# sz3/libcimbar

Hardware: NVIDIA H100
Metric: decoded cimbar frames/sec (1024x1024 mode-B) (higher is better)
Workload: dtype u8 (integer/bitwise; float32 only in the colour classifier, bit-exact vs reference)

## Files before the change

### libcimbar_b200/csrc/api.cu

```cuda
#include "ctx.cuh"
#include "k1_decode.cuh"
#include "k2_rs.cuh"
#include "render.cuh"
#include "encode.cuh"

#include <atomic>
#include <cmath>
#include <cstdio>
#include <cstring>
#include <string>
#include <vector>

using namespace cb200;

namespace {

thread_local std::string g_err;
std::atomic<unsigned long long> g_launches{0};

}
namespace cb200 {
int fail(int code, const std::string& msg) { g_err = msg; return code; }
int fail_cuda(cudaError_t e, const char* what)
{
// ... 528 lines not shown
int cb200_destroy(cb200_ctx* c)
{
    if (!c) return CB200_OK;
    cudaSetDevice(c->device);
    for (int k = 0; k < cb200_ctx::kEvSets; ++k) for (int i = 0; i < 8; ++i) if (c->ev[k][i]) cudaEventDestroy(c->ev[k][i]);
    for (const auto& s : c->stage) if (s.ev) cudaEventDestroy(s.ev);
    if (c->ccm_ev) cudaEventDestroy(c->ccm_ev);
    gather_destroy(c->gather);
    deskew_destroy(c->deskew); scan_destroy(c->scan);
    if (c->own_stream) cudaStreamDestroy(c->own_stream);
    delete c;
    return CB200_OK;
}

int cb200_get_info(const cb200_ctx* c, cb200_info* out)
{
    if (!c || !out) return fail(CB200_ERR_ARG, "null argument");
    fill_info(c->mode, c->max_frames, c->sm_count, out);
    return CB200_OK;
}

int cb200_set_stream(cb200_ctx* c, void* cuda_stream)
{
    if (!c) return fail(CB200_ERR_ARG, "null context");
    c->stream = cuda_stream ? (cudaStream_t)cuda_stream : c->own_stream;
    return CB200_OK;
}

int cb200_sync(cb200_ctx* c)
{
    if (!c) return fail(CB200_ERR_ARG, "null context");
    CK(cudaStreamSynchronize(c->stream), "cudaStreamSynchronize");
    return CB200_OK;
}

int cb200_decode_raw_dev(cb200_ctx* c, const uint8_t* d_rgb, int n, uint32_t flags, uint8_t* d_raw_out, uint8_t* d_frame_flags)
{
    int rc = check_frame_flags(flags); if (rc) return rc;
    rc = check_n(c, n); if (rc) return rc;
    if (n == 0) return CB200_OK;
    if (!d_rgb || !d_raw_out) return fail(CB200_ERR_ARG, "null buffer");
    CK(cudaSetDevice(c->device), "cudaSetDevice");
    const uint16_t* idx;
    rc = idx_for(c, flags, &idx); if (rc) return rc;
    rc = run_cells(c, d_rgb, n, flags, nullptr); if (rc) return rc;
    CK(k2_pack_launch(c->mode, c->d_cellvals, idx, n, d_raw_out, c->stream), "pack launch");
    mark(c);
    if (d_frame_flags) CK(cudaMemcpyAsync(d_frame_flags, c->d_flags, (size_t)n, cudaMemcpyDeviceToDevice, c->stream), "copy flags");
    return CB200_OK;
}

int cb200_rs_correct_dev(cb200_ctx* c, const uint8_t* d_raw, int n, uint8_t* d_data_out, uint8_t* d_block_ok)
{
    int rc = check_n(c, n); if (rc) return rc;
    if (n == 0) return CB200_OK;
    if (!d_raw || !d_data_out) return fail(CB200_ERR_ARG, "null buffer");
    CK(cudaSetDevice(c->device), "cudaSetDevice");
    uint8_t* ok = d_block_ok ? d_block_ok : c->d_ok;
    CK(k2_rs_launch(c->mode, d_raw, n, d_data_out, ok, c->d_rho, c->sm_count, c->stream), "rs launch");
    return CB200_OK;
}

}

namespace {
int decode_chunks(cb200_ctx* c, const uint8_t* d_rgb, int n, uint32_t flags, const uint8_t* sharpen, uint8_t* d_chunks,
                  uint32_t* d_chunk_mask, uint8_t* d_frame_flags, const uint8_t* d_sel_bytes = nullptr, bool enqueue_only = false)
{
    int rc = check_n(c, n); if (rc) return rc;
    if (n == 0) return CB200_OK;
    if (!d_rgb || !d_chunks || !d_chunk_mask) return fail(CB200_ERR_ARG, "null buffer");
    CK(cudaSetDevice(c->device), "cudaSetDevice");
    const Mode& m = c->mode;
    if ((flags & CB200_FLAG_CC_FIT) && (flags & CB200_FLAG_CC_SIMPLE)) return fail(CB200_ERR_ARG, "CC_SIMPLE and CC_FIT are exclusive");
    const bool fit = (flags & CB200_FLAG_CC_FIT) && !m.legacy && m.ecc_bytes > 0 && m.color_bits > 0;
    bool carried = false;
    if (enqueue_only && !(flags & CB200_FLAG_CC_SIMPLE) && c->ccm_pending) {
        const cudaError_t q = cudaEventQuery(c->ccm_ev);
        if (q == cudaErrorNotReady) carried = true;
        else if (q != cudaSuccess) return fail_cuda(q, "query ccm");
    }
    const uint16_t* idx;
    rc = idx_for(c, flags, &idx); if (rc) return rc;
    if (!fit && !carried) {
        rc = run_cells(c, d_rgb, n, flags & ~CB200_FLAG_CC_FIT, sharpen, nullptr, nullptr, d_sel_bytes); if (rc) return rc;
        mark(c);
        CK(k2_rs_fused_launch(m, c->d_cellvals, idx, n, d_chunks, c->d_ok, c->d_rho, c->sm_count, c->stream), "rs launch");
    } else {
        rc = ccm_buffers(c); if (rc) return rc;
        CK(c->d_means.ensure((size_t)c->max_frames * m.num_cells), "cudaMalloc means");
        CK(c->d_ccm_active.ensure((size_t)c->max_frames), "cudaMalloc ccm flags");
        CcmArg initial;
        if (carried) {
            memset(&initial, 0, sizeof(initial));
            initial.per_frame = c->d_carry;
            initial.per_frame_active = reinterpret_cast<const uint8_t*>(c->d_carry + 9);
        } else {
            rc = ccm_arg(c, initial); if (rc) return rc;
        }
        rc = run_cells(c, d_rgb, n, flags & ~(CB200_FLAG_CC_FIT | CB200_FLAG_CC_SIMPLE), sharpen, nullptr, c->d_means, d_sel_bytes); if (rc) return rc;
        mark(c);
        if (fit) {
            CK(k2_rs_fused_launch(m, c->d_cellvals, idx, n, d_chunks, c->d_ok, c->d_rho, c->sm_count, c->stream, 0, m.nblocks_sym), "rs launch (symbols)");
            CK(ccm_fit_launch(m, d_rgb, d_chunks, c->d_ok, idx, n, c->d_fit, c->d_fit_valid, c->stream), "ccm fit");
        } else {
            CK(cudaMemsetAsync(c->d_fit_valid, 0, (size_t)n, c->stream), "memset fit flags");
        }
        CK(ccm_carry_launch(n, c->d_fit, c->d_fit_valid, initial, c->d_ccm, c->d_ccm_active, c->stream), "ccm carry");
        CK(ccm_apply_launch(m, c->d_means, n, c->d_ccm, c->d_ccm_active, c->d_cellvals, c->stream), "ccm apply");
        if (fit) {
            CK(k2_rs_fused_launch(m, c->d_cellvals, idx, n, d_chunks, c->d_ok, c->d_rho, c->sm_count, c->stream, m.nblocks_sym, m.nblocks - m.nblocks_sym),
               "rs launch (colours)");
            rc = ccm_keep_last(c, n, c->d_ccm_active); if (rc) return rc;
        } else {
            CK(k2_rs_fused_launch(m, c->d_cellvals, idx, n, d_chunks, c->d_ok, c->d_rho, c->sm_count, c->stream), "rs launch");
        }
    }
    mark(c);
    CK(k2_mask_launch(m, c->d_ok, n, d_chunk_mask, c->stream), "mask launch");
    mark(c);
    if (d_frame_flags) CK(cudaMemcpyAsync(d_frame_flags, c->d_flags, (size_t)n, cudaMemcpyDeviceToDevice, c->stream), "copy flags");
    return CB200_OK;
}
}

extern "C" {

int cb200_decode_chunks_dev(cb200_ctx* c, const uint8_t* d_rgb, int n, uint32_t flags, uint8_t* d_chunks, uint32_t* d_chunk_mask, uint8_t* d_frame_flags)
{
    int rc = check_frame_flags(flags); if (rc) return rc;
    return decode_chunks(c, d_rgb, n, flags, nullptr, d_chunks, d_chunk_mask, d_frame_flags);
}

int cb200_decode_chunks_sharpen_dev(cb200_ctx* c, const uint8_t* d_rgb, int n, uint32_t flags, const uint8_t* sharpen, uint8_t* d_chunks,
                                    uint32_t* d_chunk_mask, uint8_t* d_frame_flags)
{
    int rc = check_selection_args(flags, sharpen); if (rc) return rc;
    return decode_chunks(c, d_rgb, n, flags, sharpen, d_chunks, d_chunk_mask, d_frame_flags);
}

int cb200_decode_raw(cb200_ctx* c, const uint8_t* rgb, int n, uint32_t flags, uint8_t* raw_out, uint8_t* frame_flags)
{
    int rc = check_frame_flags(flags); if (rc) return rc;
    rc = check_n(c, n); if (rc) return rc;
    if (n == 0) return CB200_OK;
    if (!rgb || !raw_out) return fail(CB200_ERR_ARG, "null buffer");
    CK(cudaSetDevice(c->device), "cudaSetDevice");
    rc = upload_frames(c, rgb, n); if (rc) return rc;
    rc = cb200_decode_raw_dev(c, c->d_rgb, n, flags, c->d_raw, nullptr); if (rc) return rc;
    CK(cudaMemcpyAsync(raw_out, c->d_raw, (size_t)n * c->mode.cap_all, cudaMemcpyDeviceToHost, c->stream), "D2H raw");
    if (frame_flags) CK(cudaMemcpyAsync(frame_flags, c->d_flags, (size_t)n, cudaMemcpyDeviceToHost, c->stream), "D2H flags");
    CK(cudaStreamSynchronize(c->stream), "sync");
    return CB200_OK;
}

int cb200_decode(cb200_ctx* c, const uint8_t* rgb, int n, uint32_t flags, uint8_t* data_out, uint8_t* block_ok, uint8_t* frame_flags)
{
    int rc = check_frame_flags(flags); if (rc) return rc;
    rc = check_n(c, n); if (rc) return rc;
    if (n == 0) return CB200_OK;
    if (!rgb || !data_out) return fail(CB200_ERR_ARG, "null buffer");
    CK(cudaSetDevice(c->device), "cudaSetDevice");
    rc = upload_frames(c, rgb, n); if (rc) return rc;
    rc = cb200_decode_chunks_dev(c, c->d_rgb, n, flags, c->d_data, c->d_mask, nullptr); if (rc) return rc;
    CK(cudaMemcpyAsync(data_out, c->d_data, (size_t)n * c->mode.data_bytes, cudaMemcpyDeviceToHost, c->stream), "D2H data");
    if (block_ok) CK(cudaMemcpyAsync(block_ok, c->d_ok, (size_t)n * c->mode.nblocks, cudaMemcpyDeviceToHost, c->stream), "D2H ok");
    if (frame_flags) CK(cudaMemcpyAsync(frame_flags, c->d_flags, (size_t)n, cudaMemcpyDeviceToHost, c->stream), "D2H flags");
    CK(cudaStreamSynchronize(c->stream), "sync");
    return CB200_OK;
}

}

namespace {
int decode_fountain_from_host(cb200_ctx* c, const uint8_t* rgb, int n, uint32_t flags, const uint8_t* sharpen, uint8_t* chunks_out,
                              uint32_t* chunk_count, uint32_t* chunk_mask, uint8_t* frame_flags)
{
    int rc = check_n(c, n); if (rc) return rc;
    if (n == 0) return CB200_OK;
    if (!rgb || !chunks_out || !chunk_count) return fail(CB200_ERR_ARG, "null buffer");
    CK(cudaSetDevice(c->device), "cudaSetDevice");
    rc = upload_frames(c, rgb, n); if (rc) return rc;
    return decode_fountain_to_host(c, c->d_rgb, n, flags, sharpen, chunks_out, chunk_count, chunk_mask, frame_flags);
}
}

int cb200::decode_fountain_to_host(cb200_ctx* c, const uint8_t* d_rgb, int n, uint32_t flags, const uint8_t* sharpen, uint8_t* chunks_out,
                                   uint32_t* chunk_count, uint32_t* chunk_mask, uint8_t* frame_flags)
{
    int rc = check_n(c, n); if (rc) return rc;
    if (n == 0) return CB200_OK;
    if (!d_rgb || !chunks_out || !chunk_count) return fail(CB200_ERR_ARG, "null buffer");
    CK(cudaSetDevice(c->device), "cudaSetDevice");
    rc = decode_chunks(c, d_rgb, n, flags, sharpen, c->d_data, c->d_mask, nullptr); if (rc) return rc;
    return fetch_fountain(c, n, nullptr, chunks_out, chunk_count, chunk_mask, frame_flags, nullptr);
}

int cb200::decode_chunks_enqueue(cb200_ctx* c, const uint8_t* d_rgb, int n, uint32_t flags, const uint8_t* d_sharp, uint8_t* d_chunks,
// ... 220 lines not shown
```

### libcimbar_b200/csrc/k2_rs.cu

```cuda
#include "cb200_common.cuh"
#include "k2_rs.cuh"
#include <cstring>
#include <cstdint>

namespace cb200 {

constexpr int kMaxParity = 64;

__constant__ uint8_t c_gf_exp[512];
__constant__ uint8_t c_gf_log[256];

__device__ __forceinline__ uint32_t slot_value(const uint8_t* __restrict__ cells, const uint16_t* __restrict__ idx,
                                               uint32_t s, int stream, int symbol_bits)
{
    uint32_t v = cells[idx[s]] & 0x7Fu;
    uint32_t sym_mask = (1u << symbol_bits) - 1u;
    if (stream == 0) return v & sym_mask;
    if (stream == 1) return v >> symbol_bits;
    return v;
}

__device__ __forceinline__ uint32_t stream_byte(const uint8_t* __restrict__ cells, const uint16_t* __restrict__ idx,
                                                uint32_t B, int w, int stream, int symbol_bits, uint32_t nslots)
{
// ... 320 lines not shown
#pragma unroll
                        for (int u = 0; u < kU; ++u) {
                            const int i = lane + 32 * u;
                            sl[u] = i < blk ? *reinterpret_cast<const uint2*>(idx + 4u * (B0 + (uint32_t)i - (uint32_t)m.cap_sym)) : make_uint2(0u, 0u);
                        }
                        uint32_t c0[kU], c1[kU], c2[kU], c3[kU];
#pragma unroll
                        for (int u = 0; u < kU; ++u) {
                            const int i = lane + 32 * u;
                            if (i < blk) { c0[u] = cells[sl[u].x & 0xFFFFu]; c1[u] = cells[sl[u].x >> 16]; c2[u] = cells[sl[u].y & 0xFFFFu]; c3[u] = cells[sl[u].y >> 16]; }
                            else { c0[u] = c1[u] = c2[u] = c3[u] = 0; }
                        }
#pragma unroll
                        for (int u = 0; u < kU; ++u) {
                            const int i = lane + 32 * u;
                            if (i < blk)
                                enc[i] = (uint8_t)((((c0[u] >> 4) & 3u) << 6) | (((c1[u] >> 4) & 3u) << 4) | (((c2[u] >> 4) & 3u) << 2) | ((c3[u] >> 4) & 3u));
                        }
                    }
                } else {
                    for (int i = lane; i < blk; i += 32) {
                        uint32_t B = (uint32_t)b * (uint32_t)blk + (uint32_t)i, v;
                        if (m.legacy) v = stream_byte(cells, idx, B, m.symbol_bits + m.color_bits, 2, m.symbol_bits, (uint32_t)m.num_cells);
                        else if ((int)B < m.cap_sym) v = stream_byte(cells, idx, B, m.symbol_bits, 0, m.symbol_bits, (uint32_t)m.num_cells);
                        else v = stream_byte(cells, idx, B - (uint32_t)m.cap_sym, m.color_bits, 1, m.symbol_bits, (uint32_t)m.num_cells);
                        enc[i] = (uint8_t)v;
                    }
                }
            } else {
                const uint8_t* enc_g = raw + (size_t)f * m.cap_all + (size_t)b * blk;
                for (int i = lane; i < blk; i += 32) enc[i] = enc_g[i];
            }
        }
        __syncwarp();

        uint32_t word = 0;
        {
            const int top_src = grp * GL + (Pw - 1);
#pragma unroll 2
            for (int t = 0; t < nsteps; ++t) {
                const uint32_t ew = lds_u32(stage_lane + 4u * (uint32_t)t);
                const uint32_t tw = __shfl_sync(0xffffffffu, word, top_src);
                const uint32_t v = tw ^ __byte_perm(ew, 0u, 0x0123);
                const uint32_t r0 = lds_u32(lt_lane + (((v) & 0xFFu) + 0u) * (4u * GL));
                const uint32_t r1 = lds_u32(lt_lane + (((v >> 8) & 0xFFu) + 256u) * (4u * GL));
                const uint32_t r2 = lds_u32(lt_lane + (((v >> 16) & 0xFFu) + 512u) * (4u * GL));
                const uint32_t r3 = lds_u32(lt_lane + ((v >> 24) + 768u) * (4u * GL));
                uint32_t prev = __shfl_up_sync(0xffffffffu, word, 1, GL);
                if (k == 0) prev = 0;
                word = prev ^ r0 ^ r1 ^ r2 ^ r3;
            }
        }
        const uint32_t dirty = __ballot_sync(0xffffffffu, k < Pw && word != 0u);

#pragma unroll 1
        for (int g = 0; g < G; ++g) {
            const long gb = unit * G + g;
            if (gb >= total_blocks) break;
            const int f = (int)(gb / b_count), b = b_begin + (int)(gb - (long)f * b_count);
            uint8_t* out = data_out + ((size_t)f * m.nblocks + b) * msg_len;
            uint8_t* enc = w.stage + g * kStagePitch + lead;
            if (((dirty >> (g * GL)) & ((1u << GL) - 1u)) == 0u) {
                for (int i = lane; i < msg_len; i += 32) out[i] = enc[i];
                if (lane == 0) block_ok[(size_t)f * m.nblocks + b] = 1;
                continue;
            }
            __syncwarp();
            const bool good = rs_correct_block<T>(s, w, enc, md, blk, pad, grp == g && k < Pw, word, k, lane);
            __syncwarp();
            if (!good) {
                for (int i = lane; i < msg_len; i += 32) out[i] = 0;
                if (lane == 0) block_ok[(size_t)f * m.nblocks + b] = 0;
                continue;
            }
        for (int i = lane; i < msg_len; i += 32) out[i] = enc[i];
        if (lane == 0) block_ok[(size_t)f * m.nblocks + b] = 1;
        }
    }
}

constexpr int kFrWarps = 32;
constexpr int kFrFrames = 2;
constexpr int kFrBlk = 155, kFrWords = 39, kFrPitch = 160;

struct RsFrSmem {
    static constexpr bool kSynTable = true;
    uint8_t exp[512];
    uint8_t log[256];
    struct PerWarp {
        alignas(8) uint2 masks[32];
        alignas(4) uint8_t rem[64];
        alignas(2) uint16_t remlog[kMaxParity];
        uint8_t synd[kMaxParity];
        uint8_t loc[kMaxParity + 8];
        uint8_t last[kMaxParity + 8];
        uint8_t omega[kMaxParity];
        uint8_t roots[kMaxParity + 8];
    } w[kFrWarps];
    uint8_t la[kLaDim][kLaDim];
    alignas(8) uint2 wsyn[32][32];
};

__device__ __forceinline__ void cp_async16(uint32_t dst_shared, const void* src)
{
    asm volatile("cp.async.cg.shared.global [%0], [%1], 16;" ::"r"(dst_shared), "l"(src) : "memory");
}

__global__ void __launch_bounds__(kFrWarps * 32, 2)
k_rs_frames(const Mode m, const uint8_t* __restrict__ cellvals, const uint16_t* __restrict__ idx, int n_frames,
            uint8_t* __restrict__ data_out, uint8_t* __restrict__ block_ok, const uint8_t* __restrict__ rho, int cell_pitch)
{
    constexpr int GL = 8, G = 4;
    extern __shared__ __align__(16) uint8_t rs_smem_raw[];
    RsFrSmem& s = *reinterpret_cast<RsFrSmem*>(rs_smem_raw);
    uint8_t* dyn = rs_smem_raw + ((sizeof(RsFrSmem) + 127) & ~size_t(127));
    uint32_t* lt = reinterpret_cast<uint32_t*>(dyn);
    uint8_t* cellbuf = dyn + sizeof(uint32_t) * 4 * 256 * GL;
    uint8_t* rows = cellbuf + (size_t)kFrFrames * cell_pitch;
    const int tid = threadIdx.x, warp = tid >> 5, lane = tid & 31;
    const int md = m.ecc_bytes, msg_len = m.msg_len, nb = m.nblocks, upf = nb / G;
    const int Pw = (md + 3) >> 2, pad = 4 * Pw - md;
    const int words_per_frame = nb * kFrWords, sym_rows = m.cap_sym / kFrBlk, cell_vecs = m.num_cells >> 4;
    const bool coupled6 = m.legacy != 0;
    const int n_groups = (n_frames + kFrFrames - 1) / kFrFrames;
    const uint32_t cellbuf_s = (uint32_t)__cvta_generic_to_shared(cellbuf);

    auto load_cells = [&](int gi) {
        for (int fs = 0; fs < kFrFrames; ++fs) {
            const int f = gi * kFrFrames + fs;
            if (f >= n_frames) break;
            const uint8_t* src = cellvals + (size_t)f * m.num_cells;
            for (int i = tid; i < cell_vecs; i += (int)blockDim.x) cp_async16(cellbuf_s + (uint32_t)(fs * cell_pitch + 16 * i), src + 16 * i);
        }
        asm volatile("cp.async.commit_group;" ::: "memory");
    };
    int gi = blockIdx.x;
    if (gi < n_groups) load_cells(gi);

    for (int i = tid; i < 512; i += blockDim.x) s.exp[i] = c_gf_exp[i];
    for (int i = tid; i < 256; i += blockDim.x) s.log[i] = c_gf_log[i];
    __syncthreads();
    for (int e = tid; e < md * kLaDim; e += blockDim.x) {
        const int kk = e / kLaDim, j = e % kLaDim;
        s.la[kk][j] = (uint8_t)((255 - ((j + 1) * (md - kk)) % 255) % 255);
    }
    for (int e = tid; e < 32 * 32; e += blockDim.x) {
        const int i = e >> 5, j = e & 31;
        uint2 t = make_uint2(0u, 0u);
        if (i < md && j < md) {
            const uint32_t l = (uint32_t)((255 - ((j + 1) * (md - i)) % 255) % 255);
            t.x = (uint32_t)s.exp[l] | ((uint32_t)s.exp[l + 1] << 8) | ((uint32_t)s.exp[l + 2] << 16) | ((uint32_t)s.exp[l + 3] << 24);
            t.y = (uint32_t)s.exp[l + 4] | ((uint32_t)s.exp[l + 5] << 8) | ((uint32_t)s.exp[l + 6] << 16) | ((uint32_t)s.exp[l + 7] << 24);
        }
        s.wsyn[i][j] = t;
    }
    for (int e = tid; e < 4 * 256 * GL; e += blockDim.x) {
        const int v = e / (4 * GL), j = (e / GL) & 3, kk = e % GL;
        uint32_t word = 0;
#pragma unroll
        for (int bb = 0; bb < 4; ++bb) word |= gf_mul(s, (uint32_t)v, (uint32_t)rho[j * 64 + 4 * kk + bb]) << (8 * bb);
        lt[e] = word;
    }

    RsFrSmem::PerWarp& w = s.w[warp];
    const int grp = lane / GL, k = lane % GL;
    const uint32_t lt_lane = (uint32_t)__cvta_generic_to_shared(lt) + 4u * (uint32_t)k;
    const uint32_t vsel = 0x3210u ^ (0x1111u * (uint32_t)grp);
    const uint32_t lt0 = lt_lane + 32u * (uint32_t)(0 ^ grp), lt1 = lt_lane + 32u * (uint32_t)(1 ^ grp);
    const uint32_t lt2 = lt_lane + 32u * (uint32_t)(2 ^ grp), lt3 = lt_lane + 32u * (uint32_t)(3 ^ grp);

    for (; gi < n_groups; gi += gridDim.x) {
        asm volatile("cp.async.wait_all;" ::: "memory");
        __syncthreads();
        const int nf = (n_frames - gi * kFrFrames) < kFrFrames ? (n_frames - gi * kFrFrames) : kFrFrames;

        for (int wi = tid; wi < nf * words_per_frame; wi += (int)blockDim.x) {
            const int fs = wi >= words_per_frame ? 1 : 0;
            const int rem = wi - fs * words_per_frame;
            const int r = rem / kFrWords, q = rem - r * kFrWords;
            const uint8_t* cb = cellbuf + fs * cell_pitch;
            uint32_t b0, b1, b2, b3;
            if (coupled6) {
                auto byte6 = [&](const int B) -> uint32_t {
                    const uint32_t bit0 = 8u * (uint32_t)B, sl = bit0 / 6u, skip = bit0 - 6u * sl;
                    const uint32_t v0 = cb[idx[sl]] & 63u, v1 = cb[idx[sl + 1]] & 63u;
                    return (((v0 << 6) | v1) >> (4u - skip)) & 0xFFu;
                };
                const int B0 = r * kFrBlk + 4 * q - 1;
                b0 = q ? byte6(B0) : 0u; b1 = byte6(B0 + 1); b2 = byte6(B0 + 2); b3 = byte6(B0 + 3);
            } else if (r < sym_rows) {
                const uint32_t* ix = reinterpret_cast<const uint32_t*>(idx) + (r * kFrBlk + 4 * q);
                const uint32_t i0 = q ? ix[-1] : ix[0], i1 = ix[0], i2 = ix[1], i3 = ix[2];
                b0 = ((cb[i0 & 0xFFFFu] & 15u) << 4) | (cb[i0 >> 16] & 15u);
                b1 = ((cb[i1 & 0xFFFFu] & 15u) << 4) | (cb[i1 >> 16] & 15u);
                b2 = ((cb[i2 & 0xFFFFu] & 15u) << 4) | (cb[i2 >> 16] & 15u);
                b3 = ((cb[i3 & 0xFFFFu] & 15u) << 4) | (cb[i3 >> 16] & 15u);
            } else {
                const uint2* ix = reinterpret_cast<const uint2*>(idx) + ((r - sym_rows) * kFrBlk + 4 * q);
                const uint2 i0 = q ? ix[-1] : ix[0], i1 = ix[0], i2 = ix[1], i3 = ix[2];
                auto pack = [&](const uint2 ii) {
                    return (((uint32_t)cb[ii.x & 0xFFFFu] >> 4) & 3u) << 6 | (((uint32_t)cb[ii.x >> 16] >> 4) & 3u) << 4 |
                           (((uint32_t)cb[ii.y & 0xFFFFu] >> 4) & 3u) << 2 | (((uint32_t)cb[ii.y >> 16] >> 4) & 3u);
                };
                b0 = pack(i0); b1 = pack(i1); b2 = pack(i2); b3 = pack(i3);
            }
            if (q == 0) b0 = 0;
            *reinterpret_cast<uint32_t*>(rows + (size_t)(fs * nb + r) * kFrPitch + 4 * q) = b0 | (b1 << 8) | (b2 << 16) | (b3 << 24);
        }
        __syncthreads();
        if (gi + (int)gridDim.x < n_groups) load_cells(gi + (int)gridDim.x);

        if (warp >= nf * upf) continue;
        const int fs = warp >= upf ? 1 : 0, u = warp - fs * upf, f = gi * kFrFrames + fs;
        uint8_t* urow = rows + (size_t)(fs * nb + G * u) * kFrPitch;

        uint32_t word = 0;
        {
            const uint32_t stage_lane = (uint32_t)__cvta_generic_to_shared(urow) + (uint32_t)(grp * kFrPitch);
            const int top_src = grp * GL + (Pw - 1);
#pragma unroll 3
            for (int t = 0; t < kFrWords; ++t) {
                const uint32_t ew = lds_u32(stage_lane + 4u * (uint32_t)t);
                const uint32_t tw = __shfl_sync(0xffffffffu, word, top_src);
                const uint32_t v = __byte_perm(tw ^ __byte_perm(ew, 0u, 0x0123), 0u, vsel);
                const uint32_t r0 = lds_u32(lt0 + ((v) & 0xFFu) * 128u);
                const uint32_t r1 = lds_u32(lt1 + ((v >> 8) & 0xFFu) * 128u);
                const uint32_t r2 = lds_u32(lt2 + ((v >> 16) & 0xFFu) * 128u);
                const uint32_t r3 = lds_u32(lt3 + (v >> 24) * 128u);
                uint32_t prev = __shfl_up_sync(0xffffffffu, word, 1, GL);
                if (k == 0) prev = 0;
                word = prev ^ r0 ^ r1 ^ r2 ^ r3;
            }
        }
        const uint32_t dirty = __ballot_sync(0xffffffffu, k < Pw && word != 0u);
        uint32_t okflags = 0x01010101u;
        if (dirty) {
#pragma unroll 1
            for (int g = 0; g < G; ++g) {
                if (((dirty >> (g * GL)) & ((1u << GL) - 1u)) == 0u) continue;
                uint8_t* enc = urow + g * kFrPitch + 1;
                __syncwarp();
                const bool good = rs_correct_block<1>(s, w, enc, md, kFrBlk, pad, grp == g && k < Pw, word, k, lane);
                __syncwarp();
                if (!good) {
                    for (int i = lane; i < msg_len; i += 32) enc[i] = 0;
                    okflags &= ~(1u << (8 * g));
                }
            }
            __syncwarp();
        }
        uint32_t* out32 = reinterpret_cast<uint32_t*>(data_out + ((size_t)f * nb + (size_t)(G * u)) * msg_len);
        const uint32_t urow_s = (uint32_t)__cvta_generic_to_shared(urow);
        for (int wq = lane; wq < msg_len; wq += 32) {
            const int B = 4 * wq;
            int g = (B >= msg_len) + (B >= 2 * msg_len) + (B >= 3 * msg_len);
            int i = B - g * msg_len;
            uint32_t val;
            if (i + 4 <= msg_len) {
                const uint32_t a = (uint32_t)(g * kFrPitch + 1 + i);
                const uint32_t w0 = lds_u32(urow_s + (a & ~3u)), w1 = lds_u32(urow_s + (a & ~3u) + 4u);
                val = __funnelshift_r(w0, w1, 8u * (a & 3u));
            } else {
                val = 0;
#pragma unroll
                for (int j = 0; j < 4; ++j) {
                    val |= (uint32_t)urow[g * kFrPitch + 1 + i] << (8 * j);
                    if (++i == msg_len) { i = 0; ++g; }
                }
            }
            out32[wq] = val;
        }
        if (lane == 0) *reinterpret_cast<uint32_t*>(block_ok + (size_t)f * nb + (size_t)(G * u)) = okflags;
    }
}

__global__ void k_chunk_mask(const Mode m, const uint8_t* __restrict__ block_ok, int n_frames, uint32_t* __restrict__ mask)
{
    int f = blockIdx.x * blockDim.x + threadIdx.x;
    if (f >= n_frames) return;
    const uint8_t* ok = block_ok + (size_t)f * m.nblocks;
    uint32_t out = 0;
    bool carry = false;
    for (int q = 0; q < m.chunks_per_frame; ++q) {
        bool all = true;
        for (int k = 0; k < m.blocks_per_chunk; ++k) all = all && (ok[q * m.blocks_per_chunk + k] != 0);
        if (all && !carry) out |= 1u << q;
        carry = ok[q * m.blocks_per_chunk + m.blocks_per_chunk - 1] == 0;
    }
    mask[f] = out;
}

cudaError_t k2_init_tables(const uint8_t* exp512, const uint8_t* log256)
{
    cudaError_t e = cudaMemcpyToSymbol(c_gf_exp, exp512, 512);
    if (e != cudaSuccess) return e;
    return cudaMemcpyToSymbol(c_gf_log, log256, 256);
}

cudaError_t k2_pack_launch(const Mode& m, const uint8_t* d_cellvals, const uint16_t* d_idx, int n_frames, uint8_t* d_raw, cudaStream_t st)
{
    dim3 grid((m.cap_all + 255) / 256, n_frames);
    k_pack_raw<<<grid, 256, 0, st>>>(m, d_cellvals, d_idx, n_frames, d_raw); count_launch();
    return cudaGetLastError();
}

template <int T, bool FUSED>
static cudaError_t rs_launch_t(const Mode& m, const uint8_t* d_raw, const uint8_t* d_cellvals, const uint16_t* d_idx, int n_frames,
                               uint8_t* d_data, uint8_t* d_ok, const uint8_t* d_rho, int sm_count, cudaStream_t st, int b_begin = 0, int b_count = -1)
{
    if (b_count < 0) b_count = m.nblocks;
    if (m.ecc_block + 4 > kStagePitch || m.ecc_bytes > 8 * T * 4 || m.ecc_bytes > kLaDim) return cudaErrorInvalidValue;
    const size_t smem = ((sizeof(RsSmem<T>) + 127) & ~size_t(127)) + sizeof(uint32_t) * 4 * 256 * 8 * T;
    {
        cudaError_t e = cudaFuncSetAttribute(k_rs_decode<T, FUSED>, cudaFuncAttributeMaxDynamicSharedMemorySize, (int)smem);
        if (e != cudaSuccess) return e;
    }
    const int G = 4 / T;
    long total = (long)n_frames * b_count;
    long units = (total + G - 1) / G;
    long ctas = (units + kRsWarpsPerCta - 1) / kRsWarpsPerCta;
    long max_ctas = (long)sm_count * (T == 1 ? 4 : 2);
    if (ctas > max_ctas) ctas = max_ctas;
    if (ctas < 1) ctas = 1;
    k_rs_decode<T, FUSED><<<(int)ctas, kRsWarpsPerCta * 32, smem, st>>>(m, d_raw, d_cellvals, d_idx, n_frames, b_begin, b_count, d_data, d_ok, d_rho); count_launch();
    return cudaGetLastError();
}

cudaError_t k2_rs_launch(const Mode& m, const uint8_t* d_raw, int n_frames, uint8_t* d_data, uint8_t* d_ok, const uint8_t* d_rho, int sm_count, cudaStream_t st)
{
    if (m.ecc_bytes <= 32) return rs_launch_t<1, false>(m, d_raw, nullptr, nullptr, n_frames, d_data, d_ok, d_rho, sm_count, st);
    return rs_launch_t<2, false>(m, d_raw, nullptr, nullptr, n_frames, d_data, d_ok, d_rho, sm_count, st);
}

cudaError_t k2_rs_fused_launch(const Mode& m, const uint8_t* d_cellvals, const uint16_t* d_idx, int n_frames, uint8_t* d_data,
                               uint8_t* d_ok, const uint8_t* d_rho, int sm_count, cudaStream_t st, int b_begin, int b_count)
{
    if (b_count < 0) b_count = m.nblocks;
    const bool whole = b_begin == 0 && b_count == m.nblocks;
    const bool bits_ok = m.symbol_bits == 4 && m.color_bits == 2 && (!m.legacy || (size_t)m.num_cells * 6 == (size_t)m.cap_all * 8);
    if (whole && bits_ok && m.ecc_block == kFrBlk && m.ecc_bytes <= 32 &&
        m.ecc_bytes <= kLaDim && m.nblocks % 4 == 0 && kFrFrames * (m.nblocks / 4) <= kFrWarps && m.num_cells % 16 == 0 &&
        m.cap_sym % kFrBlk == 0 && (m.nblocks * m.msg_len) % 4 == 0 && ((uintptr_t)d_data & 3u) == 0 && n_frames > 0) {
        const int cell_pitch = m.num_cells;
        const size_t smem = ((sizeof(RsFrSmem) + 127) & ~size_t(127)) + sizeof(uint32_t) * 4 * 256 * 8 +
                            (size_t)kFrFrames * cell_pitch + (size_t)kFrFrames * m.nblocks * kFrPitch;
        if (smem <= 113 * 1024) {
            cudaError_t e = cudaFuncSetAttribute(k_rs_frames, cudaFuncAttributeMaxDynamicSharedMemorySize, (int)smem);
            if (e != cudaSuccess) return e;
            int groups = (n_frames + kFrFrames - 1) / kFrFrames, ctas = groups < 2 * sm_count ? groups : 2 * sm_count;
            k_rs_frames<<<ctas, 32 * kFrFrames * (m.nblocks / 4), smem, st>>>(m, d_cellvals, d_idx, n_frames, d_data, d_ok, d_rho, cell_pitch); count_launch();
            return cudaGetLastError();
        }
    }
    if (m.ecc_bytes <= 32) return rs_launch_t<1, true>(m, nullptr, d_cellvals, d_idx, n_frames, d_data, d_ok, d_rho, sm_count, st, b_begin, b_count);
    return rs_launch_t<2, true>(m, nullptr, d_cellvals, d_idx, n_frames, d_data, d_ok, d_rho, sm_count, st, b_begin, b_count);
}

void k2_remainder_basis(const uint8_t* gen, int parity, const uint8_t* gexp512, const uint8_t* glog256, uint8_t* rho_out )
{
    const int Pw = (parity + 3) / 4, D = 4 * Pw, pad = D - parity;
    uint8_t G[72] = {0};
    for (int k = 0; k <= parity; ++k) G[pad + k] = gen[k];
    auto mul = [&](uint8_t x, uint8_t y) -> uint8_t { return (x && y) ? gexp512[glog256[x] + glog256[y]] : 0; };
    uint8_t r[64] = {0};
    r[0] = 1;
    for (int e = 1; e <= D + 3; ++e) {
        const uint8_t top = r[D - 1];
        for (int k = D - 1; k > 0; --k) r[k] = r[k - 1];
        r[0] = 0;
        if (top) for (int k = 0; k < D; ++k) r[k] ^= mul(top, G[k]);
        if (e >= D) { for (int k = 0; k < 64; ++k) rho_out[(e - D) * 64 + k] = k < D ? r[k] : 0; }
    }
}

cudaError_t k2_mask_launch(const Mode& m, const uint8_t* d_ok, int n_frames, uint32_t* d_mask, cudaStream_t st)
{
    k_chunk_mask<<<(n_frames + 127) / 128, 128, 0, st>>>(m, d_ok, n_frames, d_mask); count_launch();
    return cudaGetLastError();
}

}
```

### libcimbar_b200/csrc/k2_rs.cuh

```cuda
#pragma once
#include "cb200_common.cuh"

namespace cb200 {
cudaError_t k2_init_tables(const uint8_t* exp512, const uint8_t* log256);
cudaError_t k2_pack_launch(const Mode& m, const uint8_t* d_cellvals, const uint16_t* d_idx, int n_frames, uint8_t* d_raw, cudaStream_t st);
cudaError_t k2_rs_launch(const Mode& m, const uint8_t* d_raw, int n_frames, uint8_t* d_data, uint8_t* d_ok, const uint8_t* d_rho, int sm_count, cudaStream_t st);
void k2_remainder_basis(const uint8_t* gen, int parity, const uint8_t* gexp512, const uint8_t* glog256, uint8_t* rho_out);
cudaError_t k2_rs_fused_launch(const Mode& m, const uint8_t* d_cellvals, const uint16_t* d_idx, int n_frames, uint8_t* d_data,
                               uint8_t* d_ok, const uint8_t* d_rho, int sm_count, cudaStream_t st, int b_begin = 0, int b_count = -1);
cudaError_t k2_mask_launch(const Mode& m, const uint8_t* d_ok, int n_frames, uint32_t* d_mask, cudaStream_t st);
}
```

Before: 922,300.

## Compute interleave cell addresses arithmetically and vectorise RS syndrome staging loads

The fused Reed-Solomon kernel no longer reads the global index table to gather cells. It derives each slot's cell position arithmetically from the fixed interleave pattern (155 rows by 40 columns, two parts). Staging is reassigned so each warp lane packs the words of its own row, and the LFSR remainder loop reads four staged words at a time with 128-bit shared loads. The lookup table is built in big-endian byte order, which removes a byte swap per step. In exchange, the fast path now requires the mode's cell count to match the hard-coded interleave geometry, and the index argument is no longer used there.

Result: no change. 927,900, median of 6 (+0.6%).

```diff
diff --git a/libcimbar_b200/csrc/api.cu b/libcimbar_b200/csrc/api.cu
--- a/libcimbar_b200/csrc/api.cu
+++ b/libcimbar_b200/csrc/api.cu
@@ -634,10 +634,11 @@
     }
     const uint16_t* idx;
     rc = idx_for(c, flags, &idx); if (rc) return rc;
+    const bool interleaved = !(flags & CB200_FLAG_NO_INTERLEAVE);
     if (!fit && !carried) {
         rc = run_cells(c, d_rgb, n, flags & ~CB200_FLAG_CC_FIT, sharpen, nullptr, nullptr, d_sel_bytes); if (rc) return rc;
         mark(c);
-        CK(k2_rs_fused_launch(m, c->d_cellvals, idx, n, d_chunks, c->d_ok, c->d_rho, c->sm_count, c->stream), "rs launch");
+        CK(k2_rs_fused_launch(m, c->d_cellvals, idx, interleaved, n, d_chunks, c->d_ok, c->d_rho, c->sm_count, c->stream), "rs launch");
     } else {
         rc = ccm_buffers(c); if (rc) return rc;
         CK(c->d_means.ensure((size_t)c->max_frames * m.num_cells), "cudaMalloc means");
@@ -653,7 +654,7 @@
         rc = run_cells(c, d_rgb, n, flags & ~(CB200_FLAG_CC_FIT | CB200_FLAG_CC_SIMPLE), sharpen, nullptr, c->d_means, d_sel_bytes); if (rc) return rc;
         mark(c);
         if (fit) {
-            CK(k2_rs_fused_launch(m, c->d_cellvals, idx, n, d_chunks, c->d_ok, c->d_rho, c->sm_count, c->stream, 0, m.nblocks_sym), "rs launch (symbols)");
+            CK(k2_rs_fused_launch(m, c->d_cellvals, idx, interleaved, n, d_chunks, c->d_ok, c->d_rho, c->sm_count, c->stream, 0, m.nblocks_sym), "rs launch (symbols)");
             CK(ccm_fit_launch(m, d_rgb, d_chunks, c->d_ok, idx, n, c->d_fit, c->d_fit_valid, c->stream), "ccm fit");
         } else {
             CK(cudaMemsetAsync(c->d_fit_valid, 0, (size_t)n, c->stream), "memset fit flags");
@@ -661,11 +662,11 @@
         CK(ccm_carry_launch(n, c->d_fit, c->d_fit_valid, initial, c->d_ccm, c->d_ccm_active, c->stream), "ccm carry");
         CK(ccm_apply_launch(m, c->d_means, n, c->d_ccm, c->d_ccm_active, c->d_cellvals, c->stream), "ccm apply");
         if (fit) {
-            CK(k2_rs_fused_launch(m, c->d_cellvals, idx, n, d_chunks, c->d_ok, c->d_rho, c->sm_count, c->stream, m.nblocks_sym, m.nblocks - m.nblocks_sym),
+            CK(k2_rs_fused_launch(m, c->d_cellvals, idx, interleaved, n, d_chunks, c->d_ok, c->d_rho, c->sm_count, c->stream, m.nblocks_sym, m.nblocks - m.nblocks_sym),
                "rs launch (colours)");
             rc = ccm_keep_last(c, n, c->d_ccm_active); if (rc) return rc;
         } else {
-            CK(k2_rs_fused_launch(m, c->d_cellvals, idx, n, d_chunks, c->d_ok, c->d_rho, c->sm_count, c->stream), "rs launch");
+            CK(k2_rs_fused_launch(m, c->d_cellvals, idx, interleaved, n, d_chunks, c->d_ok, c->d_rho, c->sm_count, c->stream), "rs launch");
         }
     }
     mark(c);
diff --git a/libcimbar_b200/csrc/k2_rs.cu b/libcimbar_b200/csrc/k2_rs.cu
--- a/libcimbar_b200/csrc/k2_rs.cu
+++ b/libcimbar_b200/csrc/k2_rs.cu
@@ -426,6 +426,17 @@
 constexpr int kFrWarps = 32;
 constexpr int kFrFrames = 2;
 constexpr int kFrBlk = 155, kFrWords = 39, kFrPitch = 160;
+constexpr int kFrCols = 40;
+constexpr int kFrPart = kFrBlk * kFrCols;
+
+__device__ __forceinline__ uint32_t frame_slot_cell(uint32_t s, const bool interleaved)
+{
+    if (!interleaved) return s;
+    const uint32_t p = s >= (uint32_t)kFrPart ? (uint32_t)kFrPart : 0u;
+    s -= p;
+    const uint32_t b = s / (uint32_t)kFrCols;
+    return p + (uint32_t)kFrBlk * (s - (uint32_t)kFrCols * b) + b;
+}
 
 struct RsFrSmem {
     static constexpr bool kSynTable = true;
@@ -451,7 +462,7 @@
 }
 
 __global__ void __launch_bounds__(kFrWarps * 32, 2)
-k_rs_frames(const Mode m, const uint8_t* __restrict__ cellvals, const uint16_t* __restrict__ idx, int n_frames,
+k_rs_frames(const Mode m, const uint8_t* __restrict__ cellvals, const bool interleaved, int n_frames,
             uint8_t* __restrict__ data_out, uint8_t* __restrict__ block_ok, const uint8_t* __restrict__ rho, int cell_pitch)
 {
     constexpr int GL = 8, G = 4;
@@ -464,7 +475,7 @@
     const int tid = threadIdx.x, warp = tid >> 5, lane = tid & 31;
     const int md = m.ecc_bytes, msg_len = m.msg_len, nb = m.nblocks, upf = nb / G;
     const int Pw = (md + 3) >> 2, pad = 4 * Pw - md;
-    const int words_per_frame = nb * kFrWords, sym_rows = m.cap_sym / kFrBlk, cell_vecs = m.num_cells >> 4;
+    const int sym_rows = m.cap_sym / kFrBlk, cell_vecs = m.num_cells >> 4;
     const bool coupled6 = m.legacy != 0;
     const int n_groups = (n_frames + kFrFrames - 1) / kFrFrames;
     const uint32_t cellbuf_s = (uint32_t)__cvta_generic_to_shared(cellbuf);
@@ -502,79 +513,109 @@
         const int v = e / (4 * GL), j = (e / GL) & 3, kk = e % GL;
         uint32_t word = 0;
 #pragma unroll
-        for (int bb = 0; bb < 4; ++bb) word |= gf_mul(s, (uint32_t)v, (uint32_t)rho[j * 64 + 4 * kk + bb]) << (8 * bb);
+        for (int bb = 0; bb < 4; ++bb) word |= gf_mul(s, (uint32_t)v, (uint32_t)rho[j * 64 + 4 * kk + bb]) << (24 - 8 * bb);
         lt[e] = word;
     }
 
     RsFrSmem::PerWarp& w = s.w[warp];
     const int grp = lane / GL, k = lane % GL;
     const uint32_t lt_lane = (uint32_t)__cvta_generic_to_shared(lt) + 4u * (uint32_t)k;
-    const uint32_t vsel = 0x3210u ^ (0x1111u * (uint32_t)grp);
+    const uint32_t sel0 = 0x4440u | (3u ^ 0u ^ (uint32_t)grp), sel1 = 0x4440u | (3u ^ 1u ^ (uint32_t)grp);
+    const uint32_t sel2 = 0x4440u | (3u ^ 2u ^ (uint32_t)grp), sel3 = 0x4440u | (3u ^ 3u ^ (uint32_t)grp);
     const uint32_t lt0 = lt_lane + 32u * (uint32_t)(0 ^ grp), lt1 = lt_lane + 32u * (uint32_t)(1 ^ grp);
     const uint32_t lt2 = lt_lane + 32u * (uint32_t)(2 ^ grp), lt3 = lt_lane + 32u * (uint32_t)(3 ^ grp);
+
+    const int fs = warp >= upf ? 1 : 0, u = warp - fs * upf;
+    const int r = G * u + grp;
+    const uint8_t* cb = cellbuf + fs * cell_pitch;
+    uint8_t* urow = rows + (size_t)(fs * nb + G * u) * kFrPitch;
+    const uint32_t step = interleaved ? (uint32_t)kFrBlk : 1u;
 
     for (; gi < n_groups; gi += gridDim.x) {
         asm volatile("cp.async.wait_all;" ::: "memory");
         __syncthreads();
         const int nf = (n_frames - gi * kFrFrames) < kFrFrames ? (n_frames - gi * kFrFrames) : kFrFrames;
-
-        for (int wi = tid; wi < nf * words_per_frame; wi += (int)blockDim.x) {
-            const int fs = wi >= words_per_frame ? 1 : 0;
-            const int rem = wi - fs * words_per_frame;
-            const int r = rem / kFrWords, q = rem - r * kFrWords;
-            const uint8_t* cb = cellbuf + fs * cell_pitch;
-            uint32_t b0, b1, b2, b3;
-            if (coupled6) {
-                auto byte6 = [&](const int B) -> uint32_t {
-                    const uint32_t bit0 = 8u * (uint32_t)B, sl = bit0 / 6u, skip = bit0 - 6u * sl;
-                    const uint32_t v0 = cb[idx[sl]] & 63u, v1 = cb[idx[sl + 1]] & 63u;
-                    return (((v0 << 6) | v1) >> (4u - skip)) & 0xFFu;
-                };
+        const bool active = warp < nf * upf;
+
+        if (active) {
+#pragma unroll 1
+            for (int q = 5 * k; q < 5 * k + 5 && q < kFrWords; ++q) {
+                uint32_t b[4];
                 const int B0 = r * kFrBlk + 4 * q - 1;
-                b0 = q ? byte6(B0) : 0u; b1 = byte6(B0 + 1); b2 = byte6(B0 + 2); b3 = byte6(B0 + 3);
-            } else if (r < sym_rows) {
-                const uint32_t* ix = reinterpret_cast<const uint32_t*>(idx) + (r * kFrBlk + 4 * q);
-                const uint32_t i0 = q ? ix[-1] : ix[0], i1 = ix[0], i2 = ix[1], i3 = ix[2];
-                b0 = ((cb[i0 & 0xFFFFu] & 15u) << 4) | (cb[i0 >> 16] & 15u);
-                b1 = ((cb[i1 & 0xFFFFu] & 15u) << 4) | (cb[i1 >> 16] & 15u);
-                b2 = ((cb[i2 & 0xFFFFu] & 15u) << 4) | (cb[i2 >> 16] & 15u);
-                b3 = ((cb[i3 & 0xFFFFu] & 15u) << 4) | (cb[i3 >> 16] & 15u);
-            } else {
-                const uint2* ix = reinterpret_cast<const uint2*>(idx) + ((r - sym_rows) * kFrBlk + 4 * q);
-                const uint2 i0 = q ? ix[-1] : ix[0], i1 = ix[0], i2 = ix[1], i3 = ix[2];
-                auto pack = [&](const uint2 ii) {
-                    return (((uint32_t)cb[ii.x & 0xFFFFu] >> 4) & 3u) << 6 | (((uint32_t)cb[ii.x >> 16] >> 4) & 3u) << 4 |
-                           (((uint32_t)cb[ii.y & 0xFFFFu] >> 4) & 3u) << 2 | (((uint32_t)cb[ii.y >> 16] >> 4) & 3u);
-                };
-                b0 = pack(i0); b1 = pack(i1); b2 = pack(i2); b3 = pack(i3);
-            }
-            if (q == 0) b0 = 0;
-            *reinterpret_cast<uint32_t*>(rows + (size_t)(fs * nb + r) * kFrPitch + 4 * q) = b0 | (b1 << 8) | (b2 << 16) | (b3 << 24);
+                if (coupled6) {
+                    const int z = q == 0;
+                    const uint32_t bit0 = 8u * (uint32_t)(B0 + z), s0 = bit0 / 6u, skip = bit0 - 6u * s0;
+                    const uint32_t c0 = frame_slot_cell(s0, interleaved);
+                    uint32_t wrap = 6u, back = 0u;
+                    if (interleaved) {
+                        const uint32_t sp = s0 >= (uint32_t)kFrPart ? s0 - (uint32_t)kFrPart : s0;
+                        wrap = (uint32_t)kFrCols - sp % (uint32_t)kFrCols;
+                        back = (s0 < (uint32_t)kFrPart && sp / (uint32_t)kFrCols == (uint32_t)kFrBlk - 1u) ? (uint32_t)kFrBlk - 1u : (uint32_t)kFrPart - 1u;
+                    }
+                    uint32_t lo = 0, hi = 0;
+#pragma unroll
+                    for (int i = 0; i < 6; ++i) {
+                        const uint32_t v = cb[c0 + step * (uint32_t)i - ((uint32_t)i >= wrap ? back : 0u)] & 63u;
+                        if (i == 0) hi = v >> 2;
+                        lo |= v << (30 - 6 * i);
+                    }
+                    const uint32_t be = __funnelshift_r(lo, hi, 4u - skip);
+                    const uint32_t le = __byte_perm(be, 0u, 0x0123);
+                    b[0] = z ? 0u : le & 0xFFu; b[1] = z ? le & 0xFFu : (le >> 8) & 0xFFu;
+                    b[2] = z ? (le >> 8) & 0xFFu : (le >> 16) & 0xFFu; b[3] = z ? (le >> 16) & 0xFFu : le >> 24;
+                } else {
+                    const bool sym = r < sym_rows;
+                    const uint32_t sps = sym ? 2u : 4u;
+                    const uint32_t s1 = sps * (uint32_t)(B0 + 1 - (sym ? 0 : sym_rows * kFrBlk));
+                    const uint32_t c1 = frame_slot_cell(s1, interleaved);
+                    const uint32_t a1 = interleaved ? s1 % (uint32_t)kFrCols : 0u;
+                    const uint32_t wrapfix = interleaved ? (uint32_t)kFrPart - 1u : 0u;
+                    uint32_t c[4];
+                    c[0] = q ? c1 - step * sps + (a1 < sps ? wrapfix : 0u) : c1;
+                    c[1] = c1;
+                    c[2] = c1 + step * sps - (a1 + sps >= (uint32_t)kFrCols ? wrapfix : 0u);
+                    c[3] = c1 + 2u * step * sps - (a1 + 2u * sps >= (uint32_t)kFrCols ? wrapfix : 0u);
+#pragma unroll
+                    for (int j = 0; j < 4; ++j) {
+                        const uint32_t x = c[j];
+                        b[j] = sym ? ((cb[x] & 15u) << 4) | (cb[x + step] & 15u)
+                                   : ((((uint32_t)cb[x] >> 4) & 3u) << 6) | ((((uint32_t)cb[x + step] >> 4) & 3u) << 4) |
+                                     ((((uint32_t)cb[x + 2u * step] >> 4) & 3u) << 2) | (((uint32_t)cb[x + 3u * step] >> 4) & 3u);
+                    }
+                    if (q == 0) b[0] = 0u;
+                }
+                *reinterpret_cast<uint32_t*>(urow + grp * kFrPitch + 4 * q) = b[0] | (b[1] << 8) | (b[2] << 16) | (b[3] << 24);
+            }
         }
         __syncthreads();
         if (gi + (int)gridDim.x < n_groups) load_cells(gi + (int)gridDim.x);
 
-        if (warp >= nf * upf) continue;
-        const int fs = warp >= upf ? 1 : 0, u = warp - fs * upf, f = gi * kFrFrames + fs;
-        uint8_t* urow = rows + (size_t)(fs * nb + G * u) * kFrPitch;
+        if (!active) continue;
+        const int f = gi * kFrFrames + fs;
 
         uint32_t word = 0;
         {
-            const uint32_t stage_lane = (uint32_t)__cvta_generic_to_shared(urow) + (uint32_t)(grp * kFrPitch);
+            const uint4* stage = reinterpret_cast<const uint4*>(urow + grp * kFrPitch);
             const int top_src = grp * GL + (Pw - 1);
-#pragma unroll 3
-            for (int t = 0; t < kFrWords; ++t) {
-                const uint32_t ew = lds_u32(stage_lane + 4u * (uint32_t)t);
+            auto lfsr = [&](const uint32_t ew) {
                 const uint32_t tw = __shfl_sync(0xffffffffu, word, top_src);
-                const uint32_t v = __byte_perm(tw ^ __byte_perm(ew, 0u, 0x0123), 0u, vsel);
-                const uint32_t r0 = lds_u32(lt0 + ((v) & 0xFFu) * 128u);
-                const uint32_t r1 = lds_u32(lt1 + ((v >> 8) & 0xFFu) * 128u);
-                const uint32_t r2 = lds_u32(lt2 + ((v >> 16) & 0xFFu) * 128u);
-                const uint32_t r3 = lds_u32(lt3 + (v >> 24) * 128u);
+                const uint32_t v = tw ^ ew;
+                const uint32_t r0 = lds_u32(lt0 + (__byte_perm(v, 0u, sel0) << 7));
+                const uint32_t r1 = lds_u32(lt1 + (__byte_perm(v, 0u, sel1) << 7));
+                const uint32_t r2 = lds_u32(lt2 + (__byte_perm(v, 0u, sel2) << 7));
+                const uint32_t r3 = lds_u32(lt3 + (__byte_perm(v, 0u, sel3) << 7));
                 uint32_t prev = __shfl_up_sync(0xffffffffu, word, 1, GL);
                 if (k == 0) prev = 0;
                 word = prev ^ r0 ^ r1 ^ r2 ^ r3;
-            }
+            };
+#pragma unroll 1
+            for (int t = 0; t < kFrWords / 4; ++t) {
+                const uint4 e = stage[t];
+                lfsr(e.x); lfsr(e.y); lfsr(e.z); lfsr(e.w);
+            }
+            const uint4 e = stage[kFrWords / 4];
+            lfsr(e.x); lfsr(e.y); lfsr(e.z);
+            static_assert(kFrWords % 4 == 3, "the last four words of a row hold three staged words");
         }
         const uint32_t dirty = __ballot_sync(0xffffffffu, k < Pw && word != 0u);
         uint32_t okflags = 0x01010101u;
@@ -584,7 +625,7 @@
                 if (((dirty >> (g * GL)) & ((1u << GL) - 1u)) == 0u) continue;
                 uint8_t* enc = urow + g * kFrPitch + 1;
                 __syncwarp();
-                const bool good = rs_correct_block<1>(s, w, enc, md, kFrBlk, pad, grp == g && k < Pw, word, k, lane);
+                const bool good = rs_correct_block<1>(s, w, enc, md, kFrBlk, pad, grp == g && k < Pw, __byte_perm(word, 0u, 0x0123), k, lane);
                 __syncwarp();
                 if (!good) {
                     for (int i = lane; i < msg_len; i += 32) enc[i] = 0;
@@ -676,15 +717,15 @@
     return rs_launch_t<2, false>(m, d_raw, nullptr, nullptr, n_frames, d_data, d_ok, d_rho, sm_count, st);
 }
 
-cudaError_t k2_rs_fused_launch(const Mode& m, const uint8_t* d_cellvals, const uint16_t* d_idx, int n_frames, uint8_t* d_data,
-                               uint8_t* d_ok, const uint8_t* d_rho, int sm_count, cudaStream_t st, int b_begin, int b_count)
+cudaError_t k2_rs_fused_launch(const Mode& m, const uint8_t* d_cellvals, const uint16_t* d_idx, bool interleaved, int n_frames,
+                               uint8_t* d_data, uint8_t* d_ok, const uint8_t* d_rho, int sm_count, cudaStream_t st, int b_begin, int b_count)
 {
     if (b_count < 0) b_count = m.nblocks;
     const bool whole = b_begin == 0 && b_count == m.nblocks;
     const bool bits_ok = m.symbol_bits == 4 && m.color_bits == 2 && (!m.legacy || (size_t)m.num_cells * 6 == (size_t)m.cap_all * 8);
     if (whole && bits_ok && m.ecc_block == kFrBlk && m.ecc_bytes <= 32 &&
         m.ecc_bytes <= kLaDim && m.nblocks % 4 == 0 && kFrFrames * (m.nblocks / 4) <= kFrWarps && m.num_cells % 16 == 0 &&
-        m.cap_sym % kFrBlk == 0 && (m.nblocks * m.msg_len) % 4 == 0 && ((uintptr_t)d_data & 3u) == 0 && n_frames > 0) {
+        m.cap_sym % kFrBlk == 0 && m.num_cells == 2 * kFrPart && (m.nblocks * m.msg_len) % 4 == 0 && ((uintptr_t)d_data & 3u) == 0 && n_frames > 0) {
         const int cell_pitch = m.num_cells;
         const size_t smem = ((sizeof(RsFrSmem) + 127) & ~size_t(127)) + sizeof(uint32_t) * 4 * 256 * 8 +
                             (size_t)kFrFrames * cell_pitch + (size_t)kFrFrames * m.nblocks * kFrPitch;
@@ -692,7 +733,7 @@
             cudaError_t e = cudaFuncSetAttribute(k_rs_frames, cudaFuncAttributeMaxDynamicSharedMemorySize, (int)smem);
             if (e != cudaSuccess) return e;
             int groups = (n_frames + kFrFrames - 1) / kFrFrames, ctas = groups < 2 * sm_count ? groups : 2 * sm_count;
-            k_rs_frames<<<ctas, 32 * kFrFrames * (m.nblocks / 4), smem, st>>>(m, d_cellvals, d_idx, n_frames, d_data, d_ok, d_rho, cell_pitch); count_launch();
+            k_rs_frames<<<ctas, 32 * kFrFrames * (m.nblocks / 4), smem, st>>>(m, d_cellvals, interleaved, n_frames, d_data, d_ok, d_rho, cell_pitch); count_launch();
             return cudaGetLastError();
         }
     }
diff --git a/libcimbar_b200/csrc/k2_rs.cuh b/libcimbar_b200/csrc/k2_rs.cuh
--- a/libcimbar_b200/csrc/k2_rs.cuh
+++ b/libcimbar_b200/csrc/k2_rs.cuh
@@ -6,7 +6,8 @@
 cudaError_t k2_pack_launch(const Mode& m, const uint8_t* d_cellvals, const uint16_t* d_idx, int n_frames, uint8_t* d_raw, cudaStream_t st);
 cudaError_t k2_rs_launch(const Mode& m, const uint8_t* d_raw, int n_frames, uint8_t* d_data, uint8_t* d_ok, const uint8_t* d_rho, int sm_count, cudaStream_t st);
 void k2_remainder_basis(const uint8_t* gen, int parity, const uint8_t* gexp512, const uint8_t* glog256, uint8_t* rho_out);
-cudaError_t k2_rs_fused_launch(const Mode& m, const uint8_t* d_cellvals, const uint16_t* d_idx, int n_frames, uint8_t* d_data,
-                               uint8_t* d_ok, const uint8_t* d_rho, int sm_count, cudaStream_t st, int b_begin = 0, int b_count = -1);
+cudaError_t k2_rs_fused_launch(const Mode& m, const uint8_t* d_cellvals, const uint16_t* d_idx, bool interleaved, int n_frames,
+                               uint8_t* d_data, uint8_t* d_ok, const uint8_t* d_rho, int sm_count, cudaStream_t st, int b_begin = 0,
+                               int b_count = -1);
 cudaError_t k2_mask_launch(const Mode& m, const uint8_t* d_ok, int n_frames, uint32_t* d_mask, cudaStream_t st);
 }
```
